# fengranMark/HAConvDR

Hardware: AMD Instinct MI355X
Metric: queries/sec (encode+top-100) over N-passage 768-d corpus; HBM GB/s vs peak (higher is better)
Workload: dtype bf16 MFMA operands with fp32 accumulate / LayerNorm / softmax in the encoder (cosine vs the fp32 reference within 1e-3, measured ~1e-5); search scores and order = the fp32 fmaf chain, bit-exact

## Files before the change

haconvdr_amd/csrc/gemm8.inc:

```

enum { EPI8_QKV = 0, EPI8_RESID = 2, EPI8_GELU = 3 };
#ifndef G8_N1
#define G8_N1 4
#endif

struct Gemm8Args {
    const bf16 *A;
    const bf16 *W;
    int N, K;
    int n_groups;
    int n_tile0;
    const int *total_rows;
    const float2 *astats;
    const float *wsum;
    const float *cvec;
    bf16 *q, *k, *v16;
    const bf16 *resid;
    const float2 *rstats;
    const float *rgamma, *rbeta;
    bf16 *yb;
    float2 *part;
    bf16 *h;
    unsigned long long *clk;
    int stagger;
    int stagger_mode;
};

__device__ __forceinline__ void glds16(const bf16 *src, unsigned char *dst) {
    typedef const __attribute__((address_space(1))) void *gvp;
    typedef __attribute__((address_space(3))) void *lvp;
    __builtin_amdgcn_global_load_lds((gvp)src, (lvp)dst, 16, 0, 0);
}
__device__ __forceinline__ void swap16(unsigned &a, unsigned &b) {
    const auto r = __builtin_amdgcn_permlane16_swap(a, b, false, false);
    a = r[0];
    b = r[1];
}
__device__ __forceinline__ void quad_transpose4(f4v &v, int p) {
    int x0 = __float_as_int(v.x), x1 = __float_as_int(v.y), x2 = __float_as_int(v.z), x3 = __float_as_int(v.w);
    {
        const bool odd = p & 1;
        const int sa = odd ? x0 : x1, sb = odd ? x2 : x3;
        const int ra = __builtin_amdgcn_update_dpp(0, sa, 0xB1, 0xF, 0xF, false);
        const int rb = __builtin_amdgcn_update_dpp(0, sb, 0xB1, 0xF, 0xF, false);
        x0 = odd ? ra : x0;
        x1 = odd ? x1 : ra;
        x2 = odd ? rb : x2;
        x3 = odd ? x3 : rb;
    }
    {
        const bool hi = p & 2;
        const int sa = hi ? x0 : x2, sb = hi ? x1 : x3;
        const int ra = __builtin_amdgcn_update_dpp(0, sa, 0x4E, 0xF, 0xF, false);
        const int rb = __builtin_amdgcn_update_dpp(0, sb, 0x4E, 0xF, 0xF, false);
        x0 = hi ? ra : x0;
        x2 = hi ? x2 : ra;
        x1 = hi ? rb : x1;
        x3 = hi ? x3 : rb;
    }
    v.x = __int_as_float(x0);
    v.y = __int_as_float(x1);
    v.z = __int_as_float(x2);
    v.w = __int_as_float(x3);
}

__device__ __forceinline__ void xchg8(uint4 &a, uint4 &b, bool lo) {
    unsigned *pa = reinterpret_cast<unsigned *>(&a), *pb = reinterpret_cast<unsigned *>(&b);
#pragma unroll
    for (int i = 0; i < 4; ++i) {
        const unsigned send = lo ? pb[i] : pa[i];
        const unsigned recv = (unsigned)__builtin_amdgcn_update_dpp(0, (int)send, 0x128, 0xF, 0xF, false);
        pa[i] = lo ? pa[i] : recv;
        pb[i] = lo ? recv : pb[i];
    }
}

typedef unsigned g8_u4 __attribute__((ext_vector_type(4)));
typedef unsigned g8_u2 __attribute__((ext_vector_type(2)));
template <bool NT> __device__ __forceinline__ void g8_store16(void *p, uint4 v) {
    if constexpr (NT) __builtin_nontemporal_store(g8_u4{v.x, v.y, v.z, v.w}, reinterpret_cast<g8_u4 *>(p));
    else *reinterpret_cast<uint4 *>(p) = v;
}
template <bool NT> __device__ __forceinline__ void g8_store8(void *p, uint2 v) {
    if constexpr (NT) __builtin_nontemporal_store(g8_u2{v.x, v.y}, reinterpret_cast<g8_u2 *>(p));
    else *reinterpret_cast<uint2 *>(p) = v;
}

__device__ __forceinline__ unsigned pack_bf16(float lo, float hi) {
    typedef __bf16 bf16x2_t __attribute__((ext_vector_type(2)));
    bf16x2_t v;
    v.x = (bf16)lo;
    v.y = (bf16)hi;
    return __builtin_bit_cast(unsigned, v);
}

__device__ __forceinline__ f2v gelu8_2(f2v x) {
    f2v z = x * 0.70710678118654752f;
    z.x = __builtin_amdgcn_fmed3f(z.x, -3.0f, 3.0f);
    z.y = __builtin_amdgcn_fmed3f(z.y, -3.0f, 3.0f);
    const f2v u = z * z;
    f2v p = u * (-1.546677965e-07f) + 6.9032217e-06f;
    p = p * u + (-0.0001336812065f);
    p = p * u + 0.001487465865f;
    p = p * u + (-0.0106578986f);
    p = p * u + 0.0524059485f;
    p = p * u + (-0.1851637965f);
    p = p * u + 0.56346134f;
    return x * (z * p + 0.5f);
}

template <int EPI, bool NT>
__global__ __launch_bounds__(512, 2) void gemm8_kernel(Gemm8Args g) {
    extern __shared__ __attribute__((aligned(16))) unsigned char smem[];
    const int tid = threadIdx.x, lane = tid & 63;
    const int w = __builtin_amdgcn_readfirstlane(tid >> 6);
    const int wr = w >> 2, wc = w & 3;
    if constexpr (EPI == EPI8_GELU) {
        if (g.clk && blockIdx.x == 0 && tid == 0) {
            g.clk[0] = __builtin_amdgcn_s_memtime();
            g.clk[1] = __builtin_amdgcn_s_memrealtime();
        }
    }
    const int K = g.K, KT = K >> 6, nx = (g.N >> 8) - g.n_tile0;
    const int NG = g.n_groups, nxg = nx / NG, NP = 8 / NG;
    const int xcd = blockIdx.x & 7, slot = blockIdx.x >> 3, per_xcd = (gridDim.x + 7 - xcd) >> 3;
    const int mt_all = (*g.total_rows + 255) >> 8;
    const int mt_lo = (int)((long)mt_all * (xcd / NG) / NP), mt_hi = (int)((long)mt_all * (xcd / NG + 1) / NP);
    const int n_base = g.n_tile0 + (xcd % NG) * nxg;
    const int run_lo = 0, run_hi = (mt_hi - mt_lo) * nxg;
    const int tile0 = run_lo + slot;
    if (tile0 >= run_hi) return;
    const int my_tiles = (run_hi - tile0 + per_xcd - 1) / per_xcd;
    const int srow = lane >> 3;
    const int sch0 = (lane & 7) ^ (srow >> 1);
    const int chE = sch0 * 8, chO = (sch0 ^ 4) * 8;
    int s_tile = tile0, s_kt = 0;
    const bf16 *s_A = g.A + (size_t)((mt_lo + s_tile / nxg) << 8) * K, *s_W = g.W + (size_t)((n_base + s_tile % nxg) << 8) * K;
    const int wq = w & 3;
    const unsigned lsrcE = (unsigned)(((wr ? wq * 64 : wq * 32) + srow) * K + chE);
    const unsigned lsrcO = (unsigned)(((wr ? wq * 64 : wq * 32) + 8 + srow) * K + chO);
    const int ring_base = (wr ? 98304 : 0) + wq * 4096, ring_slots = wr ? 4 : 6;
    int h_half = 0, h_slot = 0, h_p = 0;
    const bf16 *h_base = wr ? s_W : s_A;
    long h_left = (long)my_tiles * KT * 8;
    constexpr int N1 = G8_N1, N2 = 8 - N1;
    auto issue_piece = [&]() __attribute__((always_inline)) {
        const bf16 *src = h_base + (size_t)(h_half * (wr ? 32 : 128) + (h_p >> 1) * 16) * K + s_kt * 64;
        unsigned char *dst = smem + ring_base + (h_slot << 14) + h_p * 1024;
        glds16(src + ((h_p & 1) ? lsrcO : lsrcE), dst);
        if (++h_p == 4) {
            h_p = 0;
            h_slot = h_slot + 1 == ring_slots ? 0 : h_slot + 1;
            if (++h_half == 2) {
                h_half = 0;
                if (++s_kt == KT) {
                    s_kt = 0;
                    s_tile += per_xcd;
                    h_base = wr ? g.W + (size_t)((n_base + s_tile % nxg) << 8) * K : g.A + (size_t)((mt_lo + s_tile / nxg) << 8) * K;
                }
            }
        }
    };
    auto issue_pieces = [&](auto ntag) __attribute__((always_inline)) -> bool {
        constexpr int n = decltype(ntag)::value;
        if (h_left <= 0) return false;
        h_left -= n;
#pragma unroll
        for (int i = 0; i < n; ++i) issue_piece();
        return true;
    };
    constexpr std::integral_constant<int, N1> n1tag{};
    constexpr std::integral_constant<int, 16> n16tag{};

    const int m16 = lane & 15, kg = lane >> 4, sw = (m16 >> 1) & 7;
    const int c0 = ((kg ^ sw) << 4), c1 = (((4 + kg) ^ sw) << 4);
    const int a_row = (wr * 64 + m16) * 128, w_row = (wc * 32 + m16) * 128;

#ifdef G8_STAMP
    unsigned long long stamps[16] = {0, 0, 0, 0, 0, 0, 0, 0, 0, 0, 0, 0, 0, 0, 0, 0};
    unsigned long long est[16] = {0, 0, 0, 0, 0, 0, 0, 0, 0, 0, 0, 0, 0, 0, 0, 0};
#define G8_T(i, cond) if (cond) stamps[i] = __builtin_amdgcn_s_memtime()
#define G8_E(i) if (seq == 2) est[i] = __builtin_amdgcn_s_memtime()
#else
#define G8_E(i)
#define G8_T(i, cond)
#endif
#ifdef G8_STAMP2
    unsigned long long ph[16] = {0, 0, 0, 0, 0, 0, 0, 0, 0, 0, 0, 0, 0, 0, 0, 0};
#define G8_P(i) if (seq == 3 && kt == 6) ph[i] = __builtin_amdgcn_s_memtime()
#else
#define G8_P(i)
#endif
    constexpr bool RL = EPI == EPI8_RESID;
    f32x4 acc[2][2][4][2];
    bf16x8 wf0[2][2], wf1[2][2], af0[4][2];

    issue_pieces(n16tag);
    if (g.stagger) {
        const int ph = g.stagger_mode == 0 ? (xcd & 3) : g.stagger_mode == 1 ? (slot & 3) : g.stagger_mode == 2 ? xcd : (slot & 7);
        for (int i = ph * g.stagger; i > 0; --i) __builtin_amdgcn_s_sleep(32);
    }
    asm volatile("s_waitcnt vmcnt(0)" ::: "memory");
    __builtin_amdgcn_s_barrier();

    int a_cur = 0, w_cur = 0;
    for (int seq = 0; seq < my_tiles; ++seq) {
        const int tile = tile0 + seq * per_xcd;
        const int m0 = (mt_lo + tile / nxg) << 8, n0 = (n_base + tile % nxg) << 8;
        unsigned char *R1 = smem, *R2 = smem, *R3 = smem;
        const size_t rl_tb = (size_t)m0 * H + n0;
        auto rl_issue_sb = [&](int i, int mt, unsigned char *dst) __attribute__((always_inline)) {
            int ln = lane;
            asm volatile("" : "+v"(ln));
            const unsigned lo = (unsigned)((ln & 15) * H + (ln >> 5) * 16 + ((ln >> 4) & 1) * 8);
#if defined(G8_RL_ABL) && (G8_RL_ABL & 2)
            const bf16 *src = g.resid + (size_t)(wr * 64 + i * 128 + mt * 16) * H + wc * 64 + lo;
#else
            const bf16 *src = g.resid + (rl_tb + (size_t)(wr * 64 + i * 128 + mt * 16) * H + wc * 64) + lo;
#endif
            glds16(src, dst);
            glds16(src + 32, dst + 1024);
        };
        auto rl_issue_cols = [&](unsigned char *dst) __attribute__((always_inline)) {
            int ln = lane;
            asm volatile("" : "+v"(ln));
            const unsigned so = (unsigned)((ln >> 5) * 128 + 2 * (ln & 31));
            glds16(reinterpret_cast<const bf16 *>(g.rstats + ((size_t)m0 + wr * 64) + so), dst);
            const int sel = (ln >> 4) & 3;
            const float *pc = g.cvec, *pg = g.rgamma, *pb = g.rbeta;
            asm volatile("" : "+s"(pc), "+s"(pg), "+s"(pb));
            const float *vb = pc;
            vb = sel == 1 ? pg : vb;
            vb = sel == 2 ? pb : vb;
            glds16(reinterpret_cast<const bf16 *>(vb + (n0 + wc * 64) + 4 * (ln & 15)), dst + 1024);
        };
        G8_T(2, seq == 3);
        if (wr == 1) __builtin_amdgcn_s_barrier();
#pragma unroll
        for (int i = 0; i < 2; ++i)
#pragma unroll
            for (int j = 0; j < 2; ++j)
#pragma unroll
                for (int mt = 0; mt < 4; ++mt)
#pragma unroll
                    for (int nt = 0; nt < 2; ++nt)
#pragma unroll
                        for (int e = 0; e < 4; ++e) acc[i][j][mt][nt][e] = 0.f;

        for (int kt = 0; kt < KT; ++kt) {
            G8_P(0);
            const unsigned char *kbA = smem + a_cur * 32768, *kbW = smem + 98304 + w_cur * 32768;
            const bool lastk = RL && kt == KT - 1;
            const bool live1 = (wr == 0 || kt) && h_left > 0 && !(lastk && wr == 0);
            if (live1) {
                h_left -= N1;
#pragma unroll
                for (int i = 0; i < N1; ++i) issue_piece();
            }
            if constexpr (RL) {
                if (lastk) {
                    R1 = smem + (a_cur == 0 ? 2 : a_cur - 1) * 32768 + w * 4096;
                    R3 = smem + a_cur * 32768 + w * 4096;
                    R2 = smem + 98304 + w_cur * 32768 + w * 4096;
                    rl_issue_cols(R1);
                    rl_issue_sb(0, 0, R1 + 2048);
                }
            }
            __builtin_amdgcn_sched_barrier(0);
            G8_P(12);
#pragma unroll
            for (int nt = 0; nt < 2; ++nt) {
                wf0[nt][0] = *reinterpret_cast<const bf16x8 *>(kbW + w_row + nt * 2048 + c0);
                wf0[nt][1] = *reinterpret_cast<const bf16x8 *>(kbW + w_row + nt * 2048 + c1);
                wf1[nt][0] = *reinterpret_cast<const bf16x8 *>(kbW + 16384 + w_row + nt * 2048 + c0);
                wf1[nt][1] = *reinterpret_cast<const bf16x8 *>(kbW + 16384 + w_row + nt * 2048 + c1);
            }
#pragma unroll
            for (int mt = 0; mt < 4; ++mt) {
                af0[mt][0] = *reinterpret_cast<const bf16x8 *>(kbA + a_row + mt * 2048 + c0);
                af0[mt][1] = *reinterpret_cast<const bf16x8 *>(kbA + a_row + mt * 2048 + c1);
            }
            __builtin_amdgcn_sched_barrier(0);
            G8_P(1);
            G8_P(2);
            asm volatile("s_waitcnt lgkmcnt(0)" ::: "memory");
            G8_P(3);
            __builtin_amdgcn_s_barrier();
            G8_P(4);
            G8_T(3 + (kt < 3 ? kt : 3), seq == 3 && kt < 4);
            __builtin_amdgcn_sched_barrier(0);
            __builtin_amdgcn_s_setprio(1);
#pragma unroll
            for (int ks = 0; ks < 2; ++ks)
#pragma unroll
                for (int mt = 0; mt < 4; ++mt)
#pragma unroll
                    for (int nt = 0; nt < 2; ++nt) {
                        acc[0][0][mt][nt] = __builtin_amdgcn_mfma_f32_16x16x32_bf16(wf0[nt][ks], af0[mt][ks], acc[0][0][mt][nt], 0, 0, 0);
                        acc[0][1][mt][nt] = __builtin_amdgcn_mfma_f32_16x16x32_bf16(wf1[nt][ks], af0[mt][ks], acc[0][1][mt][nt], 0, 0, 0);
                    }
            __builtin_amdgcn_s_setprio(0);
            G8_P(5);
            __builtin_amdgcn_s_barrier();
            G8_P(6);
            const bool live2 = h_left > 0 && !lastk;
            if (live2) {
                h_left -= N2;
#pragma unroll
                for (int i = 0; i < N2; ++i) issue_piece();
            }
            if constexpr (RL) {
                if (lastk) {
                    rl_issue_sb(0, 1, R2);
                    rl_issue_sb(0, 2, R2 + 2048);
                }
            }
            __builtin_amdgcn_sched_barrier(0);
            G8_P(13);
#pragma unroll
            for (int mt = 0; mt < 4; ++mt) {
                af0[mt][0] = *reinterpret_cast<const bf16x8 *>(kbA + 16384 + a_row + mt * 2048 + c0);
                af0[mt][1] = *reinterpret_cast<const bf16x8 *>(kbA + 16384 + a_row + mt * 2048 + c1);
            }
            __builtin_amdgcn_sched_barrier(0);
            G8_P(7);
            if (lastk) {
            } else if (kt) {
                if (!live2) asm volatile("s_waitcnt vmcnt(0)" ::: "memory");
                else if (wr == 0) asm volatile("s_waitcnt vmcnt(8)" ::: "memory");
                else asm volatile("s_waitcnt vmcnt(%0)" ::"n"(N2) : "memory");
            }
            asm volatile("s_waitcnt lgkmcnt(0)" ::: "memory");
            G8_P(8);
            __builtin_amdgcn_s_barrier();
            G8_P(9);
            __builtin_amdgcn_sched_barrier(0);
            __builtin_amdgcn_s_setprio(1);
#pragma unroll
            for (int ks = 0; ks < 2; ++ks)
#pragma unroll
                for (int mt = 0; mt < 4; ++mt)
#pragma unroll
                    for (int nt = 0; nt < 2; ++nt) {
                        acc[1][0][mt][nt] = __builtin_amdgcn_mfma_f32_16x16x32_bf16(wf0[nt][ks], af0[mt][ks], acc[1][0][mt][nt], 0, 0, 0);
                        acc[1][1][mt][nt] = __builtin_amdgcn_mfma_f32_16x16x32_bf16(wf1[nt][ks], af0[mt][ks], acc[1][1][mt][nt], 0, 0, 0);
                    }
            __builtin_amdgcn_s_setprio(0);
            G8_P(10);
            __builtin_amdgcn_s_barrier();
            G8_P(11);
            a_cur = a_cur == 2 ? 0 : a_cur + 1;
            w_cur ^= 1;
        }
        G8_T(8, seq == 2 && true);
        if (wr == 0) __builtin_amdgcn_s_barrier();
        G8_T(0, seq == 2);
        if constexpr (!RL) {
            if (wr == 1) issue_pieces(n1tag);
            asm volatile("s_waitcnt vmcnt(0)" ::: "memory");
        }
        G8_T(1, seq == 2);

#ifdef G8_NO_EPI
#pragma unroll
        for (int i = 0; i < 2; ++i)
#pragma unroll
            for (int j = 0; j < 2; ++j)
#pragma unroll
                for (int mt = 0; mt < 4; ++mt)
#pragma unroll
                    for (int nt = 0; nt < 2; ++nt) asm volatile("" ::"v"(acc[i][j][mt][nt]));
        continue;
#endif
        {
            const int colg = 8 * ((kg & 1) * 2 + (kg >> 1));
            if constexpr (RL) {
                const bool lo8 = m16 < 8;
                const unsigned lane_b = (unsigned)((wr * 64 + (m16 & 7)) * H + wc * 64 + (m16 >> 3) * 32 + colg);
                const unsigned rd_off = (unsigned)(((kg >> 1) * 16 + m16) * 16);
                const bool rd_hi = kg & 1;
#define G8_VM(n) asm volatile("s_waitcnt vmcnt(" #n ")" ::: "memory")
#define G8_VMC(c, a, b) do { if (c) G8_VM(a); else G8_VM(b); } while (0)
#define G8_LDS_DONE() asm volatile("s_waitcnt lgkmcnt(0)" ::: "memory")
                constexpr std::integral_constant<int, -1> cnone{};
                constexpr std::integral_constant<int, 0> c0t{};
                constexpr std::integral_constant<int, 1> c1t{};
                constexpr std::integral_constant<int, 2> c2t{};
                constexpr std::integral_constant<int, 3> c3t{};
                constexpr std::integral_constant<int, 8> n8tag{};
                rl_issue_sb(0, 3, R3);
                rl_issue_sb(1, 0, R3 + 2048);
                G8_E(0);
                G8_VM(8);
                G8_E(1);
                float mean_[2][4], rstd_[2][4];
                f4v rg[2][2], rb[2][2];
#pragma unroll
                for (int i = 0; i < 2; ++i)
#pragma unroll
                    for (int mt = 0; mt < 4; ++mt) {
                        g8_u4 c = *reinterpret_cast<const g8_u4 *>(R1 + i * 512 + (mt * 16 + (m16 & 14)) * 8);
                        asm volatile("" : "+v"(c));
                        asm volatile("v_mov_b32 %0, %1" : "=v"(mean_[i][mt]) : "v"((m16 & 1) ? c.z : c.x));
                        asm volatile("v_mov_b32 %0, %1" : "=v"(rstd_[i][mt]) : "v"((m16 & 1) ? c.w : c.y));
                    }
#pragma unroll
                for (int jj = 0; jj < 2; ++jj)
#pragma unroll
                    for (int nt = 0; nt < 2; ++nt) {
                        const int co = (jj * 32 + nt * 16 + 4 * kg) * 4;
                        const f4v cvv = *reinterpret_cast<const f4v *>(R1 + 1024 + co);
#pragma unroll
                        for (int i = 0; i < 2; ++i)
#pragma unroll
                            for (int mt = 0; mt < 4; ++mt) acc[i][jj][mt][nt] += cvv;
                        rg[jj][nt] = *reinterpret_cast<const f4v *>(R1 + 1024 + 256 + co);
                        rb[jj][nt] = *reinterpret_cast<const f4v *>(R1 + 1024 + 512 + co);
                    }
                auto sb_read = [&](const unsigned char *sb, g8_u4 (&c)[2][2]) __attribute__((always_inline)) {
#pragma unroll
                    for (int jj = 0; jj < 2; ++jj) {
                        c[jj][0] = *reinterpret_cast<const g8_u4 *>(sb + jj * 1024 + rd_off);
                        c[jj][1] = *reinterpret_cast<const g8_u4 *>(sb + jj * 1024 + 512 + rd_off);
                        asm volatile("" : "+v"(c[jj][0]), "+v"(c[jj][1]));
                    }
                };
                auto sb_do = [&](auto itag, auto mttag, unsigned char *sb, auto refilltag, const g8_u4 (*pre)[2]) __attribute__((always_inline)) {
                    constexpr int i = decltype(itag)::value, mt = decltype(mttag)::value, refill = decltype(refilltag)::value;
                    const float mean = mean_[i][mt], rstd = rstd_[i][mt];
                    uint4 ro[2];
                    float s1 = 0.f, s2 = 0.f;
                    g8_u4 cc[2][2];
                    if (pre) {
#pragma unroll
                        for (int jj = 0; jj < 2; ++jj) cc[jj][0] = pre[jj][0], cc[jj][1] = pre[jj][1];
                    } else {
                        sb_read(sb, cc);
                    }
#pragma unroll
                    for (int jj = 0; jj < 2; ++jj) {
                        const g8_u4 c0 = cc[jj][0], c1 = cc[jj][1];
                        const uint2 w0 = {rd_hi ? c0.z : c0.x, rd_hi ? c0.w : c0.y}, w1 = {rd_hi ? c1.z : c1.x, rd_hi ? c1.w : c1.y};
                        const f4v ra = {__uint_as_float(w0.x << 16), __uint_as_float(w0.x & 0xffff0000u), __uint_as_float(w0.y << 16), __uint_as_float(w0.y & 0xffff0000u)};
                        const f4v rb_ = {__uint_as_float(w1.x << 16), __uint_as_float(w1.x & 0xffff0000u), __uint_as_float(w1.y << 16), __uint_as_float(w1.y & 0xffff0000u)};
                        const f4v o0 = acc[i][jj][mt][0] + ((ra - mean) * rstd * rg[jj][0] + rb[jj][0]);
                        const f4v o1 = acc[i][jj][mt][1] + ((rb_ - mean) * rstd * rg[jj][1] + rb[jj][1]);
                        unsigned p0 = pack_bf16(o0.x, o0.y), p1 = pack_bf16(o0.z, o0.w);
                        unsigned p2 = pack_bf16(o1.x, o1.y), p3 = pack_bf16(o1.z, o1.w);
                        swap16(p0, p2);
                        swap16(p1, p3);
                        ro[jj] = make_uint4(p0, p1, p2, p3);
                        const f4v sm = o0 + o1, sq = o0 * o0 + o1 * o1;
                        const float t1 = (sm.x + sm.y) + (sm.z + sm.w), t2 = (sq.x + sq.y) + (sq.z + sq.w);
                        s1 = jj ? s1 + t1 : t1;
                        s2 = jj ? s2 + t2 : t2;
                    }
                    s1 += __shfl_xor(s1, 16);
                    s2 += __shfl_xor(s2, 16);
                    s1 += __shfl_xor(s1, 32);
                    s2 += __shfl_xor(s2, 32);
                    xchg8(ro[0], ro[1], lo8);
                    G8_LDS_DONE();
                    if constexpr (refill >= 0) rl_issue_sb(1, refill, sb);
                    __builtin_amdgcn_sched_barrier(0);
                    const size_t row = (size_t)m0 + i * 128 + wr * 64 + mt * 16 + m16;
#if defined(G8_RL_ABL) && (G8_RL_ABL & 1)
                    if (lane == 0) g.part[row * (g.N >> 6) + (n0 >> 6) + wc] = make_float2(s1, s2);
#pragma unroll
                    for (int jj = 0; jj < 2; ++jj)
                        if (lane == 0) g8_store16<NT>(g.yb + rl_tb + (size_t)((i * 128 + mt * 16 + jj * 8) * H) + lane_b, ro[jj]);
#else
                    if (kg == 0) g.part[row * (g.N >> 6) + (n0 >> 6) + wc] = make_float2(s1, s2);
#pragma unroll
                    for (int jj = 0; jj < 2; ++jj)
                        g8_store16<NT>(g.yb + rl_tb + (size_t)((i * 128 + mt * 16 + jj * 8) * H) + lane_b, ro[jj]);
#endif
                    __builtin_amdgcn_sched_barrier(0);
                };
                __builtin_amdgcn_sched_barrier(0);
                bool gA = false, gW = false;
                sb_do(c0t, c0t, R1 + 2048, cnone, nullptr);
                G8_E(2);
                __builtin_amdgcn_s_barrier();
                if (wr == 0) gA = issue_pieces(n8tag);
                __builtin_amdgcn_sched_barrier(0);
                G8_E(3);
                G8_VMC(gA, 17, 9);
                G8_E(4);
                sb_do(c0t, c1t, R2, c1t, nullptr);
                G8_VMC(gA, 20, 12);
                G8_E(5);
                sb_do(c0t, c2t, R2 + 2048, c2t, nullptr);
                G8_VMC(gA, 23, 15);
                G8_E(6);
                sb_do(c0t, c3t, R3, c3t, nullptr);
                G8_VMC(gA, 26, 18);
                G8_E(7);
                sb_do(c1t, c0t, R3 + 2048, cnone, nullptr);
                G8_VM(16);
                G8_E(8);
                sb_do(c1t, c1t, R2, cnone, nullptr);
                G8_VM(14);
                G8_E(9);
                sb_do(c1t, c2t, R2 + 2048, cnone, nullptr);
                G8_E(10);
                G8_VM(12);
                G8_E(11);
                g8_u4 c7[2][2];
                sb_read(R3, c7);
                G8_LDS_DONE();
                __builtin_amdgcn_s_barrier();
                if (wr == 1) gW = issue_pieces(n8tag);
                __builtin_amdgcn_sched_barrier(0);
                G8_E(12);
                sb_do(c1t, c3t, R3, cnone, c7);
                G8_E(13);
                G8_VMC(gW, 3, 27);
                G8_E(14);
                G8_E(15);
#undef G8_VM
#undef G8_VMC
#undef G8_LDS_DONE
            } else {
                float2 st[2][4];
#pragma unroll
                for (int i = 0; i < 2; ++i)
#pragma unroll
                    for (int mt = 0; mt < 4; ++mt) st[i][mt] = g.astats[(size_t)m0 + i * 128 + wr * 64 + mt * 16 + m16];
                const int ldo = EPI == EPI8_GELU ? g.N : H;
                const bool lo8 = m16 < 8;
                const unsigned lane_b = (unsigned)((wr * 64 + (m16 & 7)) * ldo + wc * 64 + (m16 >> 3) * 32 + colg);
                f4v ws[2][2], cv[2][2];
#pragma unroll
                for (int j = 0; j < 2; ++j)
#pragma unroll
                    for (int nt = 0; nt < 2; ++nt) {
                        const int nb = n0 + wc * 64 + j * 32;
                        cv[j][nt] = *reinterpret_cast<const f4v *>(g.cvec + nb + nt * 16 + 4 * kg);
                        ws[j][nt] = *reinterpret_cast<const f4v *>(g.wsum + nb + nt * 16 + 4 * kg);
                    }
#pragma unroll
                for (int i = 0; i < 2; ++i)
#pragma unroll
                    for (int mt = 0; mt < 4; ++mt) {
                        const float nm = -st[i][mt].x * st[i][mt].y;
                        float rs = st[i][mt].y;
                        asm volatile("v_mov_b32 %0, %1" : "=v"(rs) : "v"(st[i][mt].y));
                        uint4 o[2];
#pragma unroll
                        for (int j = 0; j < 2; ++j) {
                            const int nb = n0 + wc * 64 + j * 32;
                            unsigned p[4];
#pragma unroll
                            for (int nt = 0; nt < 2; ++nt) {
                                f4v v = acc[i][j][mt][nt] * rs + (ws[j][nt] * nm + cv[j][nt]);
                                if (EPI == EPI8_QKV && n0 >= 2 * H) {
                                    quad_transpose4(v, lane & 3);
                                    const int n = nb + nt * 16 + 4 * kg + (lane & 3) - 2 * H;
                                    const size_t mg = (size_t)(m0 + i * 128 + wr * 64 + mt * 16) >> 4;
                                    uint2 o2;
                                    o2.x = pack_bf16(v.x, v.y);
                                    o2.y = pack_bf16(v.z, v.w);
                                    g8_store8<NT>(g.v16 + (mg * H + n) * 16 + (m16 & 12), o2);
                                    continue;
                                }
                                if constexpr (EPI == EPI8_GELU) {
                                    const f2v g0 = gelu8_2((f2v){v.x, v.y}), g1 = gelu8_2((f2v){v.z, v.w});
                                    p[2 * nt] = pack_bf16(g0.x, g0.y);
                                    p[2 * nt + 1] = pack_bf16(g1.x, g1.y);
                                } else {
                                    p[2 * nt] = pack_bf16(v.x, v.y);
                                    p[2 * nt + 1] = pack_bf16(v.z, v.w);
                                }
                            }
                            if (EPI == EPI8_QKV && n0 >= 2 * H) continue;
                            swap16(p[0], p[2]);
                            swap16(p[1], p[3]);
                            o[j] = make_uint4(p[0], p[1], p[2], p[3]);
                        }
                        if (EPI == EPI8_QKV && n0 >= 2 * H) continue;
                        xchg8(o[0], o[1], lo8);
                        const size_t ur = (size_t)(m0 + i * 128 + mt * 16) * ldo;
#pragma unroll
                        for (int j = 0; j < 2; ++j) {
                            if constexpr (EPI == EPI8_GELU) {
                                g8_store16<NT>(g.h + ur + (size_t)(j * 8) * ldo + n0 + lane_b, o[j]);
                            } else {
                                bf16 *dst = n0 < H ? g.q + ur + n0 : g.k + ur + (n0 - H);
                                g8_store16<NT>(dst + (size_t)(j * 8) * ldo + lane_b, o[j]);
                            }
                        }
                    }
            }
        }
    }
    if constexpr (EPI == EPI8_GELU) {
        if (g.clk && blockIdx.x == 0 && tid == 0) {
            g.clk[2] = __builtin_amdgcn_s_memtime();
            g.clk[3] = __builtin_amdgcn_s_memrealtime();
        }
    }
#ifdef G8_STAMP2
    if (blockIdx.x == 8 && lane == 0 && (w == 0 || w == 4)) {
        unsigned long long *o = reinterpret_cast<unsigned long long *>(g.part) + 64 + (w ? 16 : 0);
        for (int i = 0; i < 16; ++i) o[i] = ph[i];
    }
#endif
#ifdef G8_STAMP
    if (blockIdx.x == 8 && lane == 0 && (w == 0 || w == 4)) {
        unsigned long long *o = reinterpret_cast<unsigned long long *>(g.part) + (w ? 16 : 0);
        for (int i = 0; i < 16; ++i) o[i] = stamps[i];
        for (int i = 0; i < 16; ++i) o[32 + i] = est[i];
    }
#endif
}

__global__ __launch_bounds__(256) void ln_combine_kernel(const float2 *__restrict__ part, int n_part, int n_cols, const int *__restrict__ total_rows,
                                                         float eps, float2 *__restrict__ stats) {
    const size_t row = (size_t)blockIdx.x * 256 + threadIdx.x;
    if (row >= (size_t)((*total_rows + 255) & ~255)) return;
    float s1 = 0.f, s2 = 0.f;
    if ((n_part & 1) == 0) {
        const float4 *p4 = reinterpret_cast<const float4 *>(part + row * n_part);
        float4 v[8];
        const int n4 = n_part >> 1;
#pragma unroll
        for (int i = 0; i < 8; ++i) v[i] = i < n4 ? p4[i] : make_float4(0.f, 0.f, 0.f, 0.f);
#pragma unroll
        for (int i = 0; i < 8; ++i) {
            s1 += v[i].x + v[i].z;
            s2 += v[i].y + v[i].w;
        }
        for (int i = 16; i < n_part; ++i) {
            const float2 p = part[row * n_part + i];
            s1 += p.x;
            s2 += p.y;
        }
    } else {
        for (int i = 0; i < n_part; ++i) {
            const float2 p = part[row * n_part + i];
            s1 += p.x;
            s2 += p.y;
        }
    }
    const float mean = s1 / n_cols;
    const float var = fmaxf(s2 / n_cols - mean * mean, 0.f);
    stats[row] = make_float2(mean, rsqrtf(var + eps));
}

__global__ __launch_bounds__(256) void fold_ln_kernel(const float *__restrict__ Wf, const float *__restrict__ bias, const float *__restrict__ gamma,
                                                      const float *__restrict__ beta, int K, float scale, bf16 *__restrict__ Wb,
                                                      float *__restrict__ wsum, float *__restrict__ cvec) {
    __shared__ float red[2][4];
    const int n = blockIdx.x, tid = threadIdx.x;
    float s = 0.f, c = 0.f;
    for (int k = tid; k < K; k += 256) {
        const float wv = Wf[(size_t)n * K + k];
        const bf16 wb = (bf16)(wv * (gamma ? gamma[k] : 1.f) * scale);
        Wb[(size_t)n * K + k] = wb;
        s += (float)wb;
        if (beta) c += beta[k] * wv;
    }
    s = wave_sum(s);
    c = wave_sum(c);
    if ((tid & 63) == 0) {
        red[0][tid >> 6] = s;
        red[1][tid >> 6] = c;
    }
    __syncthreads();
    if (tid == 0) {
        wsum[n] = gamma ? (red[0][0] + red[0][1]) + (red[0][2] + red[0][3]) : 0.f;
        cvec[n] = (bias[n] + (red[1][0] + red[1][1]) + (red[1][2] + red[1][3])) * scale;
    }
}

__global__ void fill_identity_stats_kernel(float2 *__restrict__ stats, size_t n) {
    const size_t i = (size_t)blockIdx.x * blockDim.x + threadIdx.x;
    if (i < n) stats[i] = make_float2(0.f, 1.f);
}
```

Measured before the change: 8256.

## Prefetch epilogue stats and column vectors into LDS during last K step

For the non-residual epilogues (QKV and GELU), the per-row LayerNorm stats and the per-column cvec/wsum vectors are now loaded asynchronously into a spare LDS region during the final K iteration. Previously each lane read them from global memory after the main loop. The next tile's pieces (n1tag) are now issued after the epilogue's LDS reads rather than before it, so those loads overlap the epilogue math and stores, with adjusted vmcnt waits. The cost is extra LDS traffic, more complex waitcnt accounting that is sensitive to outstanding-load counts, and a new barrier inside the epilogue.

```diff
diff --git a/haconvdr_amd/csrc/gemm8.inc b/haconvdr_amd/csrc/gemm8.inc
--- a/haconvdr_amd/csrc/gemm8.inc
+++ b/haconvdr_amd/csrc/gemm8.inc
@@ -192,6 +192,11 @@
 #define G8_P(i)
 #endif
     constexpr bool RL = EPI == EPI8_RESID;
+#ifdef G8_NO_EPI
+    constexpr bool EIL = false;
+#else
+    constexpr bool EIL = !RL;
+#endif
     f32x4 acc[2][2][4][2];
     bf16x8 wf0[2][2], wf1[2][2], af0[4][2];
 
@@ -234,6 +239,16 @@
             vb = sel == 2 ? pb : vb;
             glds16(reinterpret_cast<const bf16 *>(vb + (n0 + wc * 64) + 4 * (ln & 15)), dst + 1024);
         };
+        auto ei_issue = [&](unsigned char *dst) __attribute__((always_inline)) {
+            int ln = lane;
+            asm volatile("" : "+v"(ln));
+            const unsigned so = (unsigned)((ln >> 5) * 128 + 2 * (ln & 31));
+            glds16(reinterpret_cast<const bf16 *>(g.astats + ((size_t)m0 + wr * 64) + so), dst);
+            const float *pc = g.cvec, *pw = g.wsum;
+            asm volatile("" : "+s"(pc), "+s"(pw));
+            const float *vb = (ln & 16) ? pw : pc;
+            glds16(reinterpret_cast<const bf16 *>(vb + (n0 + wc * 64) + 4 * (ln & 15)), dst + 1024);
+        };
         G8_T(2, seq == 3);
         if (wr == 1) __builtin_amdgcn_s_barrier();
 #pragma unroll
@@ -247,6 +262,8 @@
 #pragma unroll
                         for (int e = 0; e < 4; ++e) acc[i][j][mt][nt][e] = 0.f;
 
+        [[maybe_unused]] int ei_kt = KT - 1;
+        if constexpr (EIL) asm volatile("" : "+s"(ei_kt));
         for (int kt = 0; kt < KT; ++kt) {
             G8_P(0);
             const unsigned char *kbA = smem + a_cur * 32768, *kbW = smem + 98304 + w_cur * 32768;
@@ -315,6 +332,11 @@
                     rl_issue_sb(0, 2, R2 + 2048);
                 }
             }
+            bool eik = false;
+            if constexpr (EIL) {
+                eik = kt == ei_kt;
+                if (eik) ei_issue(smem + 98304 + w_cur * 32768 + 16384 + w * 2048);
+            }
             __builtin_amdgcn_sched_barrier(0);
             G8_P(13);
 #pragma unroll
@@ -325,6 +347,10 @@
             __builtin_amdgcn_sched_barrier(0);
             G8_P(7);
             if (lastk) {
+            } else if (EIL && kt && eik) {
+                if (!live2) asm volatile("s_waitcnt vmcnt(2)" ::: "memory");
+                else if (wr == 0) asm volatile("s_waitcnt vmcnt(10)" ::: "memory");
+                else asm volatile("s_waitcnt vmcnt(%0)" ::"n"(N2 + 2) : "memory");
             } else if (kt) {
                 if (!live2) asm volatile("s_waitcnt vmcnt(0)" ::: "memory");
                 else if (wr == 0) asm volatile("s_waitcnt vmcnt(8)" ::: "memory");
@@ -355,7 +381,7 @@
         G8_T(8, seq == 2 && true);
         if (wr == 0) __builtin_amdgcn_s_barrier();
         G8_T(0, seq == 2);
-        if constexpr (!RL) {
+        if constexpr (!RL && !EIL) {
             if (wr == 1) issue_pieces(n1tag);
             asm volatile("s_waitcnt vmcnt(0)" ::: "memory");
         }
@@ -522,11 +548,15 @@
 #undef G8_VMC
 #undef G8_LDS_DONE
             } else {
+                const unsigned char *EI = smem + 98304 + (w_cur ^ 1) * 32768 + 16384 + w * 2048;
+                G8_E(0);
+                asm volatile("s_waitcnt vmcnt(0)" ::: "memory");
+                G8_E(1);
                 float2 st[2][4];
 #pragma unroll
                 for (int i = 0; i < 2; ++i)
 #pragma unroll
-                    for (int mt = 0; mt < 4; ++mt) st[i][mt] = g.astats[(size_t)m0 + i * 128 + wr * 64 + mt * 16 + m16];
+                    for (int mt = 0; mt < 4; ++mt) st[i][mt] = *reinterpret_cast<const float2 *>(EI + i * 512 + (mt * 16 + m16) * 8);
                 const int ldo = EPI == EPI8_GELU ? g.N : H;
                 const bool lo8 = m16 < 8;
                 const unsigned lane_b = (unsigned)((wr * 64 + (m16 & 7)) * ldo + wc * 64 + (m16 >> 3) * 32 + colg);
@@ -535,10 +565,16 @@
                 for (int j = 0; j < 2; ++j)
 #pragma unroll
                     for (int nt = 0; nt < 2; ++nt) {
-                        const int nb = n0 + wc * 64 + j * 32;
-                        cv[j][nt] = *reinterpret_cast<const f4v *>(g.cvec + nb + nt * 16 + 4 * kg);
-                        ws[j][nt] = *reinterpret_cast<const f4v *>(g.wsum + nb + nt * 16 + 4 * kg);
-                    }
+                        const int co = (j * 32 + nt * 16 + 4 * kg) * 4;
+                        cv[j][nt] = *reinterpret_cast<const f4v *>(EI + 1024 + co);
+                        ws[j][nt] = *reinterpret_cast<const f4v *>(EI + 1024 + 256 + co);
+                    }
+                asm volatile("s_waitcnt lgkmcnt(0)" ::: "memory");
+                __builtin_amdgcn_s_barrier();
+                bool gW = false;
+                if (wr == 1) gW = issue_pieces(n1tag);
+                __builtin_amdgcn_sched_barrier(0);
+                G8_E(2);
 #pragma unroll
                 for (int i = 0; i < 2; ++i)
 #pragma unroll
@@ -591,6 +627,12 @@
                             }
                         }
                     }
+                G8_E(3);
+                if (gW) {
+                    if (EPI == EPI8_QKV && n0 >= 2 * H) asm volatile("s_waitcnt vmcnt(32)" ::: "memory");
+                    else asm volatile("s_waitcnt vmcnt(16)" ::: "memory");
+                }
+                G8_E(4);
             }
         }
     }
```

After: 8241. No clear change (-0.2%).
